# TheoCoombes/ClipCap

Measured on AMD Instinct MI355X. Metric: train samples/sec (512-d prefix, 40-tok caption), higher is better.
Workload: dtype bf16; 1 GPU; BASELINE configs[1]: TransformerMapper(8L,P=L=10,H=8)+frozen GPT-2-small; per_gpu_batch=256, global_batch=256, encoder_dim=512, train_language_model=False, parallelism=dp1

## Files before the change

### clipcap_amd/csrc/gemm.hip.h

```cpp
#pragma once
#include <cstdlib>
#include <type_traits>
#include "common.hip.h"
#include "gemm_api.h"

namespace CC_NS {

constexpr int G_BM = 128, G_BN = 128, G_BK = 64, G_THREADS = 256;
constexpr int G_TILE_BYTES = G_BM * G_BK * 2;
constexpr int G_EPI_LD = 68;

struct GemmShape {
    int M, N, K;
    int lda, ldb;
    int k_chunk;
    int group_m;
    int stagger;
    int flags = 0;
};

__device__ __forceinline__ int g_lds_off(int row, int chunk) {
    return row * 128 + (((chunk ^ (row >> 1) ^ ((row >> 4) & 3)) & 7) << 4);
}

// ... 23 lines not shown
__device__ __forceinline__ void g_load_ks(StageRegs& s, const op16_t* __restrict__ base, int ld, int rows, int r0,
                                          int k0, int kend, int tid) {
    const int ng = (tid & 7) | (((tid >> 4) & 1) << 3);
    const int kg = ((tid >> 3) & 1) | ((tid >> 5) << 1);
    const int r = r0 + ng * 8;
#pragma unroll
    for (int j = 0; j < 4; j++) {
        const int k = k0 + kg * 4 + j;
        if (k < kend && r < rows)
            s.v[j] = *reinterpret_cast<const uint4*>(base + (size_t)k * ld + r);
        else
            s.v[j] = make_uint4(0, 0, 0, 0);
    }
}
__device__ __forceinline__ void l_store_ks(const StageRegs& s, char* lds, int tid) {
    const int ng = (tid & 7) | (((tid >> 4) & 1) << 3);
    const int kg = ((tid >> 3) & 1) | ((tid >> 5) << 1);
    const int kc = kg >> 1, half = (kg & 1) * 8;
    const unsigned in[4][4] = {{s.v[0].x, s.v[0].y, s.v[0].z, s.v[0].w},
                               {s.v[1].x, s.v[1].y, s.v[1].z, s.v[1].w},
                               {s.v[2].x, s.v[2].y, s.v[2].z, s.v[2].w},
                               {s.v[3].x, s.v[3].y, s.v[3].z, s.v[3].w}};
#pragma unroll
    for (int c = 0; c < 4; c++) {
        uint2 ev, od;
        ev.x = __builtin_amdgcn_perm(in[1][c], in[0][c], 0x05040100u);
        ev.y = __builtin_amdgcn_perm(in[3][c], in[2][c], 0x05040100u);
        od.x = __builtin_amdgcn_perm(in[1][c], in[0][c], 0x07060302u);
        od.y = __builtin_amdgcn_perm(in[3][c], in[2][c], 0x07060302u);
        const int n = ng * 8 + 2 * c;
        *reinterpret_cast<uint2*>(lds + g_lds_off(n, kc) + half) = ev;
        *reinterpret_cast<uint2*>(lds + g_lds_off(n + 1, kc) + half) = od;
    }
}

template <int L>
__device__ __forceinline__ void g_load(StageRegs& s, const op16_t* base, int ld, int rows, int r0, int k0, int kend,
                                       int tid) {
    if constexpr (L == 0)
        g_load_kc(s, base, ld, rows, r0, k0, kend, tid);
    else
        g_load_ks(s, base, ld, rows, r0, k0, kend, tid);
}
template <int L>
__device__ __forceinline__ void l_store(const StageRegs& s, char* lds, int tid) {
    if constexpr (L == 0)
        l_store_kc(s, lds, tid);
    else
        l_store_ks(s, lds, tid);
}


template <class E> struct epi_row_strip { static constexpr bool value = false; };
template <class E, class = void> struct epi_acc_init { static constexpr bool value = false; };
template <class E> struct epi_acc_init<E, decltype((void)&E::init4)> { static constexpr bool value = true; };
template <class E, class = void> struct epi_strip_aux { static constexpr bool value = false; typedef char type; };
template <class E> struct epi_strip_aux<E, decltype((void)sizeof(typename E::StripAux))> { static constexpr bool value = true; typedef typename E::StripAux type; };

template <class Epi, int I0 = 0, int I1 = 4>
__device__ __forceinline__ void gemm_epilogue(f32x4 (&acc)[4][4], char* smem, int wave, int lane, int row0, int col0, const Epi& epi) {
    float* strip = reinterpret_cast<float*>(smem) + wave * (16 * G_EPI_LD);
    const int er = (lane >> 4) * 4, ec = lane & 15;
    constexpr bool kAux = epi_strip_aux<Epi>::value;
    typename epi_strip_aux<Epi>::type aux[4][2];
    (void)aux;
    if constexpr (kAux) {
#pragma unroll
        for (int i = I0; i < I1; i++)
#pragma unroll
            for (int s = 0; s < 2; s++) {
                const int q = lane + 64 * s;
                aux[i][s] = epi.load_aux(row0 + i * 16 + (q >> 3), col0 + (q & 7) * 8);
            }
        __builtin_amdgcn_sched_barrier(0);
    }
#pragma unroll
    for (int i = I0; i < I1; i++) {
#pragma unroll
        for (int j = 0; j < 4; j++)
#pragma unroll
            for (int r = 0; r < 4; r++) strip[(er + r) * G_EPI_LD + j * 16 + ec] = acc[i][j][r];
#pragma unroll
        for (int s = 0; s < 2; s++) {
            const int q = lane + 64 * s;
            const int lr = q >> 3, c8 = q & 7;
            float v[8];
            const float4 a = *reinterpret_cast<const float4*>(strip + lr * G_EPI_LD + c8 * 8);
            const float4 b = *reinterpret_cast<const float4*>(strip + lr * G_EPI_LD + c8 * 8 + 4);
            v[0] = a.x; v[1] = a.y; v[2] = a.z; v[3] = a.w; v[4] = b.x; v[5] = b.y; v[6] = b.z; v[7] = b.w;
            if constexpr (kAux) epi(row0 + i * 16 + lr, col0 + c8 * 8, v, aux[i][s]);
            else epi(row0 + i * 16 + lr, col0 + c8 * 8, v);
        }
    }
}

template <class Epi, int NI, int NJ>
__device__ __forceinline__ void gemm_epilogue_regs(f32x4 (&acc)[NI][NJ], int lane, int row0, int col0, const Epi& epi) {
    static_assert(NI % 2 == 0 || NJ % 2 == 0, "leftover column tiles pair along i");
    const int q = lane >> 4, rl = lane & 15;
#define G_PAIR(X, Y, V)                                                                                                  \
    _Pragma("unroll") for (int r_ = 0; r_ < 4; r_++) {                                                                   \
        const auto s_ = __builtin_amdgcn_permlane16_swap(__float_as_uint((X)[r_]), __float_as_uint((Y)[r_]), false, false); \
        (V)[r_] = __uint_as_float(s_[0]);                                                                                \
        (V)[4 + r_] = __uint_as_float(s_[1]);                                                                            \
    }
    if constexpr (epi_row_strip<Epi>::value) {
        static_assert(!epi_row_strip<Epi>::value || NJ == 4, "row-strip epilogues need a 64-column wave strip");
        typename Epi::RowAux tg[NI];
#pragma unroll
        for (int i = 0; i < NI; i++) tg[i] = epi.load_row(row0 + i * 16 + rl);
#pragma unroll
        for (int i = 0; i < NI; i++) {
            float va[8], vb[8];
            G_PAIR(acc[i][0], acc[i][1], va);
            G_PAIR(acc[i][NJ - 2], acc[i][NJ - 1], vb);
            const int cb = col0 + (q & 1) * 16 + (q >> 1) * 8;
            epi.strip(row0 + i * 16 + rl, cb, cb + 32, va, vb, tg[i]);
        }
    } else {
        if constexpr (Epi::kPre) {
#pragma unroll
            for (int i = 0; i < NI; i++)
#pragma unroll
                for (int j = 0; j < NJ; j++) epi.pre4(row0 + i * 16 + rl, col0 + j * 16 + q * 4, acc[i][j]);
        }
        float bias[(NJ + 1) / 2][8];
#pragma unroll
        for (int jp = 0; jp < NJ / 2; jp++) epi.bias8(col0 + (2 * jp + (q & 1)) * 16 + (q >> 1) * 8, bias[jp]);
        if constexpr (NJ & 1) epi.bias8(col0 + (NJ - 1) * 16 + (q >> 1) * 8, bias[NJ / 2]);
        __builtin_amdgcn_sched_barrier(0);
#pragma unroll
        for (int i = 0; i < NI; i++) {
#pragma unroll
            for (int jp = 0; jp < NJ / 2; jp++) {
                float v[8];
                G_PAIR(acc[i][2 * jp], acc[i][2 * jp + 1], v);
                epi.fin(row0 + i * 16 + rl, col0 + (2 * jp + (q & 1)) * 16 + (q >> 1) * 8, v, bias[jp]);
            }
            if constexpr (NJ & 1) {
                if (i & 1) {
                    float v[8];
                    G_PAIR(acc[i - 1][NJ - 1], acc[i][NJ - 1], v);
                    epi.fin(row0 + (i - 1 + (q & 1)) * 16 + rl, col0 + (NJ - 1) * 16 + (q >> 1) * 8, v, bias[NJ / 2]);
                }
            }
        }
    }
#undef G_PAIR
}

__device__ __forceinline__ void tile_coords(int tile, int tiles_m, int tiles_n, int G, int& tm, int& tn) {
    const int band = tile / (G * tiles_n);
    const int first = band * G;
    const int gm = min(G, tiles_m - first);
    const int r = tile - band * G * tiles_n;
    tm = first + r % gm;
    tn = r / gm;
}

__device__ __forceinline__ void acc_zero(f32x4 (&acc)[4][4]) {
#pragma unroll
    for (int i = 0; i < 4; i++)
#pragma unroll
        for (int j = 0; j < 4; j++) acc[i][j] = f32x4{0.f, 0.f, 0.f, 0.f};
}

template <int AL, int BL, class Epi>
__global__ __launch_bounds__(G_THREADS, 2) void gemm_bf16_kernel(const op16_t* __restrict__ A,
                                                                  const op16_t* __restrict__ B, GemmShape g, Epi epi) {
    __shared__ __attribute__((aligned(16))) char smem[4 * G_TILE_BYTES];
    const int tid = threadIdx.x, lane = tid & 63, wave = tid >> 6;
    const int wm = wave >> 1, wn = wave & 1;
    const int tiles_n = (g.N + G_BN - 1) / G_BN, tiles_m = (g.M + G_BM - 1) / G_BM;
// ... 768 lines not shown
                const float* src = part + ((pw * 4 + tile) * 16 + reg) * 64 + ls;
                const float4 x = *reinterpret_cast<const float4*>(src), y = *reinterpret_cast<const float4*>(src + 4);
                v[0] += x.x; v[1] += x.y; v[2] += x.z; v[3] += x.w; v[4] += y.x; v[5] += y.y; v[6] += y.z; v[7] += y.w;
            }
            epi(m0 + row, n0 + c8 * 8, v);
        }
    }
}
static __global__ __launch_bounds__(256) void k_skinny_image(const op16_t* __restrict__ W, op16_t* __restrict__ img, int N, int K) {
    const size_t total = (size_t)N * K / 8;
    const int ktot = K / 64;
    for (size_t e = (size_t)blockIdx.x * 256 + threadIdx.x; e < total; e += (size_t)gridDim.x * 256) {
        const int l = (int)(e & 63);
        size_t f = e >> 6;
        const int i = (int)(f & 1); f >>= 1;
        const int w = (int)(f & 3); f >>= 2;
        const int kt = (int)(f % ktot), tn = (int)(f / ktot);
        const op16_t* src = W + (size_t)(tn * 64 + i * 32 + (l & 31)) * K + kt * 64 + w * 16 + (l >> 5) * 8;
        reinterpret_cast<kb_u32x4*>(img)[e] = *reinterpret_cast<const kb_u32x4*>(src);
    }
}

#endif

#ifndef CC_STAG_READ_FIRST
#define CC_STAG_READ_FIRST 1
#endif
constexpr int H_BM = 256, H_BN = 256, H_BK = 32, H_NS = 4, H_STAGE = (H_BM + H_BN) * H_BK * 2;
__device__ __forceinline__ int h_swz(int row) { return (row & 8) ? 3 : 0; }
__device__ __forceinline__ int h_lds_off(int row, int chunk) { return row * 64 + ((chunk ^ h_swz(row)) << 4); }
__device__ __forceinline__ int h_tt_g(int k) { return (k & 3) | (((k >> 3) & 1) << 2); }
#define H_ISSUE(T, IS_A)                                                                                                 \
    {                                                                                                                    \
        char* st_ = smem + ((T) % H_NS) * SSTAGE + ((IS_A) ? 0 : SBM * H_BK * 2);                                      \
        int k0_ = kbeg + (T)*H_BK;                                                                                       \
        if constexpr (X3F) k0_ = (x3c0_ + ((T) >> 1)) * H_BK + (((T) & 1) ? ((IS_A) ? 2 * x3k_ : x3k_) : 0);    \
        _Pragma("unroll") for (int i_ = 0; i_ < ((IS_A) ? (NI + 1) / 2 : NJ); i_++) {                                        \
            const int seg = (IS_A) ? min(wn + 4 * i_, 2 * NI - 1) : wn + 4 * i_;    \
            const op16_t* src;                                                                                           \
            if constexpr (TT) {                                                                                          \
                const int kr = seg * 2 + (lane >> 5);                                  \
                const int c = (lane & 31) ^ (h_tt_g(kr) << 1);                                                            \
                src = (IS_A) ? A + (size_t)(k0_ + kr) * g.lda + min(m0 + c * 8, g.M - 8)                                  \
                             : B + (size_t)(k0_ + kr) * g.ldb + min(n0 + c * 8, g.N - 8);                                 \
            } else {                                                                                                     \
                const int row = seg * 16 + (lane >> 2);                                   \
                const int chunk = (lane & 3) ^ h_swz(row);                                                               \
                src = (IS_A) ? A + (size_t)min(m0 + row, g.M - 1) * g.lda + k0_ + chunk * 8                               \
                             : B + (size_t)min(n0 + row, g.N - 1) * g.ldb + k0_ + chunk * 8;                              \
            }                                                                                                            \
            __builtin_amdgcn_global_load_lds((gptr_t)src, (lptr_t)(st_ + seg * 1024), 16, 0, 0);                         \
        }                                                                                                                \
    }
typedef __attribute__((ext_vector_type(2))) int h_i32x2;
struct HTTFrag { h_i32x2 lo, hi; };
__device__ __forceinline__ HTTFrag h_tt_read(const char* tile, int lane_base, int xoff) {
    typedef __attribute__((address_space(3))) const char* lp_t;
    const unsigned a = (unsigned)(size_t)(lp_t)(tile + lane_base + xoff);
    HTTFrag f;
    asm volatile("ds_read_b64_tr_b16 %0, %1" : "=v"(f.lo) : "v"(a) : "memory");
    asm volatile("ds_read_b64_tr_b16 %0, %1 offset:2048" : "=v"(f.hi) : "v"(a) : "memory");
    return f;
}
__device__ __forceinline__ op16x8 h_tt_oper(const HTTFrag& f) {
    typedef __attribute__((ext_vector_type(4))) int i32x4_t;
    const i32x4_t v = {f.lo[0], f.lo[1], f.hi[0], f.hi[1]};
    return __builtin_bit_cast(op16x8, v);
}
#define H_LOADF(T)                                                                                                       \
    {                                                                                                                    \
        const char* ca_ = smem + ((T) % H_NS) * SSTAGE;                                                                 \
        const char* cb_ = ca_ + SBM * H_BK * 2;                                                                         \
        if constexpr (TT) {                                                                                              \
            _Pragma("unroll") for (int i_ = 0; i_ < NI; i_++) taf[i_] = h_tt_read(ca_, tt_base, ((grp * 16 + 2 * i_) ^ tt_gx) << 4);  \
            _Pragma("unroll") for (int j_ = 0; j_ < NJ; j_++) tbf[j_] = h_tt_read(cb_, tt_base, ((wn * 8 + 2 * j_) ^ tt_gx) << 4);  \
        } else {                                                                                                         \
            _Pragma("unroll") for (int i_ = 0; i_ < NI; i_++) af[i_] = *reinterpret_cast<const op16x8*>(ca_ + h_lds_off(arow + i_ * 16 + frow, fchunk)); \
            _Pragma("unroll") for (int j_ = 0; j_ < NJ; j_++) bfr[j_] = *reinterpret_cast<const op16x8*>(cb_ + h_lds_off(bcol + j_ * 16 + frow, fchunk)); \
        }                                                                                                                \
    }
#define H_MFMA(T)                                                                                                        \
    {                                                                                                      \
        if constexpr (TT) {                                                                                              \
            _Pragma("unroll") for (int i_ = 0; i_ < NI; i_++) af[i_] = h_tt_oper(taf[i_]);                                 \
            _Pragma("unroll") for (int j_ = 0; j_ < NJ; j_++) bfr[j_] = h_tt_oper(tbf[j_]);                               \
        }                                                                                                                \
        __builtin_amdgcn_s_setprio(1);                                                                                   \
        _Pragma("unroll") for (int i_ = 0; i_ < NI; i_++) _Pragma("unroll") for (int j_ = 0; j_ < NJ; j_++)                \
            acc[i_][j_] = CC_MFMA_16x16x32(bfr[j_], af[i_], acc[i_][j_]);                \
        __builtin_amdgcn_s_setprio(0);                                                                                   \
    }
#define H_LOADF_LO(T)                                                                                                    \
    {                                                                                                                    \
        const char* ca_ = smem + ((T) % H_NS) * SSTAGE;                                                                 \
        const char* cb_ = ca_ + SBM * H_BK * 2;                                                                         \
        _Pragma("unroll") for (int i_ = 0; i_ < NI; i_++) af2[X3F ? i_ : 0] = *reinterpret_cast<const op16x8*>(ca_ + h_lds_off(arow + i_ * 16 + frow, fchunk)); \
        _Pragma("unroll") for (int j_ = 0; j_ < NJ; j_++) bf2[X3F ? j_ : 0] = *reinterpret_cast<const op16x8*>(cb_ + h_lds_off(bcol + j_ * 16 + frow, fchunk)); \
    }
#define H_MFMA_LO()                                                                                                      \
    {                                                                                                                    \
        __builtin_amdgcn_s_setprio(1);                                                                                   \
        _Pragma("unroll") for (int i_ = 0; i_ < NI; i_++) _Pragma("unroll") for (int j_ = 0; j_ < NJ; j_++)                \
            acc[i_][j_] = CC_MFMA_16x16x32(bf2[X3F ? j_ : 0], af[i_], acc[i_][j_]);                                        \
        _Pragma("unroll") for (int i_ = 0; i_ < NI; i_++) _Pragma("unroll") for (int j_ = 0; j_ < NJ; j_++)                \
            acc[i_][j_] = CC_MFMA_16x16x32(bfr[j_], af2[X3F ? i_ : 0], acc[i_][j_]);                                       \
        __builtin_amdgcn_s_setprio(0);                                                                                   \
    }
#define H_SEGEND()                                                                                                       \
    {                                                                                                                    \
        asm volatile("s_waitcnt lgkmcnt(0)" ::: "memory");                                                               \
        __builtin_amdgcn_sched_barrier(0);                                                                               \
        __builtin_amdgcn_s_barrier();                                                                                    \
        __builtin_amdgcn_sched_barrier(0);                                                                               \
    }
#define H_WAIT(T, CNT)                                                                                                   \
    {                                                                                                                    \
        const int rem_ = min(nk - 1, (T) + H_NS - 1) - ((T) + 1);                                                        \
        if (rem_ >= 3) s_wait_vm<3 * (CNT)>();                                                                           \
        else if (rem_ == 2) s_wait_vm<2 * (CNT)>();                                                                      \
        else if (rem_ == 1) s_wait_vm<(CNT)>();                                                                          \
        else s_wait_vm<0>();                                                                                             \
    }
#ifdef CC_STAMP
__device__ unsigned long long cc_stamp_buf[2 * 8];
#define H_STAMP_DECL unsigned long long st_last_ = __builtin_readcyclecounter(), st_acc_[8] = {0, 0, 0, 0, 0, 0, 0, 0};
#define H_STAMP(I) { const unsigned long long n_ = __builtin_readcyclecounter(); st_acc_[I] += n_ - st_last_; st_last_ = n_; }
#define H_STAMP_OUT if (blockIdx.x == 7 && wn == 0 && lane == 0) { for (int i_ = 0; i_ < 8; i_++) cc_stamp_buf[grp * 8 + i_] = st_acc_[i_]; }
#else
#define H_STAMP_DECL
#define H_STAMP(I)
#define H_STAMP_OUT
#endif
template <class Epi, int NJ, bool TT, int NI = 8, bool X3F = false>
__device__ __forceinline__ void gemm_stag256_body(const op16_t* __restrict__ A, const op16_t* __restrict__ B, const GemmShape& g, const Epi& epi,
                                                  int tile, int zslice, char* smem) {
    static_assert(NJ >= 2 && NJ <= 4 && (NI == 8 || NI == 10 || (NI == 5 && NJ == 4)), "wave tile is (16 NI) x (16 NJ)");
    static_assert(!TT || (NJ == 4 && NI == 8), "the K-strided image is laid out for 256 x 256 tiles");
    static_assert(!X3F || (!TT && NJ == 3 && NI == 8), "the fused split-bf16 form is the 256 x 192 NT kernel's");
    constexpr int BN = 64 * NJ, SBM = 32 * NI, SSTAGE = (SBM + H_BN) * H_BK * 2;
    const int tid = threadIdx.x, lane = tid & 63;
    const int wave = __builtin_amdgcn_readfirstlane(tid >> 6);
    const int grp = wave >> 2, wn = wave & 3;
    const int arow = grp * (16 * NI), bcol = wn * (16 * NJ);
    const int tiles_n = (g.N + BN - 1) / BN, tiles_m = (g.M + SBM - 1) / SBM;
    int tm, tn;
    tile_coords(tile, tiles_m, tiles_n, g.group_m, tm, tn);
    const int m0 = tm * SBM, n0 = tn * BN;
    const int kbeg = zslice * g.k_chunk;
    const int x3k_ = g.K / 3;
    const int x3nc_ = x3k_ / H_BK, x3per_ = (x3nc_ + (int)gridDim.z - 1) / (int)gridDim.z;
    const int x3c0_ = zslice * x3per_, x3c1_ = min(x3nc_, x3c0_ + x3per_);
    (void)x3c0_;
    const int nk = X3F ? 2 * max(0, x3c1_ - x3c0_) : (min(g.K, kbeg + g.k_chunk) - kbeg) / H_BK;
    f32x4 acc[NI][NJ];
#pragma unroll
    for (int i = 0; i < NI; i++)
#pragma unroll
        for (int j = 0; j < NJ; j++) acc[i][j] = f32x4{0.f, 0.f, 0.f, 0.f};
    constexpr bool kAccInit = epi_acc_init<Epi>::value && ((NJ == 3 && NI == 8) || NI == 5) && !X3F;
    if constexpr (kAccInit) {
        if (zslice == 0 && epi.init_from_input()) {
            const int q_ = lane >> 4, rl_ = lane & 15;
#pragma unroll
            for (int i = 0; i < NI; i++)
#pragma unroll
                for (int j = 0; j < NJ; j++) epi.init4(m0 + arow + i * 16 + rl_, n0 + bcol + j * 16 + q_ * 4, acc[i][j]);
        }
    }
    op16x8 af[NI], bfr[NJ];
    op16x8 af2[X3F ? NI : 1], bf2[X3F ? NJ : 1];
    (void)af2; (void)bf2;
    HTTFrag taf[TT ? NI : 1], tbf[TT ? NJ : 1];
    (void)taf; (void)tbf;
    const int frow = lane & 15, fchunk = lane >> 4;
    const int tt_base = (8 * fchunk + (frow >> 2)) * 512 + ((frow & 3) >> 1) * 16 + (frow & 1) * 8;
    const int tt_gx = h_tt_g(8 * fchunk + (frow >> 2)) << 1;
    (void)tt_base; (void)tt_gx;
    H_STAMP_DECL
    if constexpr (X3F) {
#define H_G0_STEP(T, LOADF, MFMA)                                                                                        \
        {                                                                                                                \
            LOADF(T);                                                                                                    \
            __builtin_amdgcn_sched_barrier(0);                                                                           \
            if ((T) + H_NS - 1 < nk) H_ISSUE((T) + H_NS - 1, true);                                                      \
            H_SEGEND();                                                                                                  \
            MFMA;                                                                                                        \
            H_WAIT(T, (NI + 1) / 2);                                                                                           \
            H_SEGEND();                                                                                                  \
        }
#define H_G1_STEP(T, LOADF, MFMA_PREV)                                                                                   \
        {                                                                                                                \
            MFMA_PREV;                                                                                                   \
            H_SEGEND();                                                                                                  \
            LOADF(T);                                                                                                    \
            __builtin_amdgcn_sched_barrier(0);                                                                           \
            if ((T) + H_NS - 1 < nk) H_ISSUE((T) + H_NS - 1, false);                                                     \
            H_WAIT(T, NJ);                                                                                               \
            H_SEGEND();                                                                                                  \
        }
        if (grp == 0) {
            if (nk > 0) H_ISSUE(0, true);
            if (nk > 1) H_ISSUE(1, true);
            if (nk > 2) H_ISSUE(2, true);
            H_WAIT(-1, (NI + 1) / 2);
            H_SEGEND();
            for (int t = 0; t < nk; t += 2) {
                H_G0_STEP(t, H_LOADF, H_MFMA(t))
                H_G0_STEP(t + 1, H_LOADF_LO, H_MFMA_LO())
            }
            H_SEGEND();
        } else {
            if (nk > 0) H_ISSUE(0, false);
            if (nk > 1) H_ISSUE(1, false);
            if (nk > 2) H_ISSUE(2, false);
            H_WAIT(-1, NJ);
            H_SEGEND();
            for (int t = 0; t < nk; t += 2) {
                H_G1_STEP(t, H_LOADF, if (t >= 1) H_MFMA_LO())
                H_G1_STEP(t + 1, H_LOADF_LO, H_MFMA(t))
            }
            if (nk > 0) H_MFMA_LO();
            H_SEGEND();
        }
#undef H_G0_STEP
#undef H_G1_STEP
    } else
    if (grp == 0) {
        H_ISSUE(0, true);
        if (nk > 1) H_ISSUE(1, true);
        if (nk > 2) H_ISSUE(2, true);
        if (H_NS > 4 && nk > 3) H_ISSUE(3, true);
        H_WAIT(-1, (NI + 1) / 2);
        H_SEGEND();
        H_STAMP(0)
        for (int t = 0; t < nk; t++) {
#if CC_STAG_READ_FIRST
            H_LOADF(t);
            __builtin_amdgcn_sched_barrier(0);
            if (t + H_NS - 1 < nk) H_ISSUE(t + H_NS - 1, true);
            H_STAMP(1)
#else
            if (t + H_NS - 1 < nk) H_ISSUE(t + H_NS - 1, true);
            H_STAMP(1)
            H_LOADF(t);
#endif
#ifdef CC_STAMP
            asm volatile("s_waitcnt lgkmcnt(0)" ::: "memory");
#endif
            H_STAMP(2)
            H_SEGEND();
            H_STAMP(3)
            H_MFMA(t);
            H_STAMP(4)
            H_WAIT(t, (NI + 1) / 2);
            H_STAMP(5)
            H_SEGEND();
            H_STAMP(6)
        }
        H_SEGEND();
    } else {
        H_ISSUE(0, false);
        if (nk > 1) H_ISSUE(1, false);
        if (nk > 2) H_ISSUE(2, false);
        if (H_NS > 4 && nk > 3) H_ISSUE(3, false);
        H_WAIT(-1, NJ);
        H_SEGEND();
        H_STAMP(0)
        for (int t = 0; t < nk; t++) {
            if (t >= 1) H_MFMA(t - 1);
            H_STAMP(4)
            H_SEGEND();
            H_STAMP(6)
#if CC_STAG_READ_FIRST
            H_LOADF(t);
            __builtin_amdgcn_sched_barrier(0);
            if (t + H_NS - 1 < nk) H_ISSUE(t + H_NS - 1, false);
            H_STAMP(1)
#else
            if (t + H_NS - 1 < nk) H_ISSUE(t + H_NS - 1, false);
            H_STAMP(1)
            H_LOADF(t);
#endif
#ifdef CC_STAMP
            asm volatile("s_waitcnt lgkmcnt(0)" ::: "memory");
#endif
            H_STAMP(2)
            H_WAIT(t, NJ);
            H_STAMP(5)
            H_SEGEND();
            H_STAMP(3)
        }
        H_MFMA(nk - 1); H_SEGEND();
    }
    H_STAMP(0)
    if constexpr (epi_acc_init<Epi>::value && !kAccInit) {
        Epi e2 = epi;
        e2.acc_init = false;
        gemm_epilogue_regs<Epi, NI, NJ>(acc, lane, m0 + arow, n0 + bcol, e2);
    } else {
        gemm_epilogue_regs<Epi, NI, NJ>(acc, lane, m0 + arow, n0 + bcol, epi);
    }
    H_STAMP(7)
    H_STAMP_OUT
}
template <class Epi, int NJ, bool TT = false, int NI = 8, bool X3F = false>
__global__ __launch_bounds__(512, 1) void gemm_nt_stag256_kernel(const op16_t* __restrict__ A, const op16_t* __restrict__ B, GemmShape g, Epi epi) {
    extern __shared__ __attribute__((aligned(1024))) char smem[];
    gemm_stag256_body<Epi, NJ, TT, NI, X3F>(A, B, g, epi, xcd_remap(blockIdx.x, gridDim.x), (int)blockIdx.z, smem);
}
#undef H_STAMP_DECL
#undef H_STAMP
#undef H_STAMP_OUT
#undef H_ISSUE
#undef H_LOADF
#undef H_MFMA
#undef H_LOADF_LO
#undef H_MFMA_LO
#undef H_SEGEND
#undef H_WAIT

#include "gemm_q4.hip.h"

__device__ __forceinline__ HTTFrag g_tt_read(const char* tile, int lane_base, int xoff) {
    typedef __attribute__((address_space(3))) const char* lp_t;
    const unsigned a = (unsigned)(size_t)(lp_t)(tile + lane_base + xoff);
    HTTFrag f;
    asm volatile("ds_read_b64_tr_b16 %0, %1" : "=v"(f.lo) : "v"(a) : "memory");
    asm volatile("ds_read_b64_tr_b16 %0, %1 offset:1024" : "=v"(f.hi) : "v"(a) : "memory");
    return f;
}
__device__ __forceinline__ void glds_tile_tt(const op16_t* __restrict__ base, int ld, int cols, int c0, int k0, char* lds, int wave, int lane) {
#pragma unroll
    for (int i = 0; i < 4; i++) {
        const int seg = wave + 4 * i;
        const int kr = seg * 4 + (lane >> 4);
        const int c = (lane & 15) ^ (h_tt_g(kr) << 1);
        const op16_t* src = base + (size_t)(k0 + kr) * ld + min(c0 + c * 8, cols - 8);
        __builtin_amdgcn_global_load_lds((gptr_t)src, (lptr_t)(lds + seg * 1024), 16, 0, 0);
    }
}
template <class Epi>
__device__ __forceinline__ void gemm_tt_glds4_body(const op16_t* __restrict__ A, const op16_t* __restrict__ B, const GemmShape& g, const Epi& epi,
                                                   int tile, int zslice, char* smemt) {
    const int tid = threadIdx.x, lane = tid & 63;
    const int wave = __builtin_amdgcn_readfirstlane(tid >> 6);
    const int wm = wave >> 1, wn = wave & 1;
    const int tiles_n = (g.N + G_BN - 1) / G_BN, tiles_m = (g.M + G_BM - 1) / G_BM;
    int tm, tn;
    tile_coords(tile, tiles_m, tiles_n, g.group_m, tm, tn);
    const int m0 = tm * G_BM, n0 = tn * G_BN;
    const int kbeg = zslice * g.k_chunk;
    const int nk = (min(g.K, kbeg + g.k_chunk) - kbeg) / G_BK;
    f32x4 acc[4][4];
#pragma unroll
    for (int i = 0; i < 4; i++)
#pragma unroll
        for (int j = 0; j < 4; j++) acc[i][j] = f32x4{0.f, 0.f, 0.f, 0.f};
#define GT_ISSUE(T)                                                                                                      \
    {                                                                                                                    \
        char* st_ = smemt + ((T) & 3) * 2 * G_TILE_BYTES;                                                                \
        glds_tile_tt(A, g.lda, g.M, m0, kbeg + (T)*G_BK, st_, wave, lane);                                               \
        glds_tile_tt(B, g.ldb, g.N, n0, kbeg + (T)*G_BK, st_ + G_TILE_BYTES, wave, lane);                                \
    }
    GT_ISSUE(0);
    if (nk > 1) GT_ISSUE(1);
    if (nk > 2) GT_ISSUE(2);
// ... 266 lines not shown
        *reinterpret_cast<float4*>(p) = make_float4(v[0] + b[0], v[1] + b[1], v[2] + b[2], v[3] + b[3]);
        *reinterpret_cast<float4*>(p + 4) = make_float4(v[4] + b[4], v[5] + b[5], v[6] + b[6], v[7] + b[7]);
    }
};

template <int ACT = -1>
struct EpiDActT {
    act_t* C;
    const act_t* aux;
    int ldc, M, Ns;
    int act;
    int img = 0;
    __device__ __forceinline__ int act_() const { return ACT >= 0 ? ACT : act; }
    __device__ __forceinline__ void operator()(int row, int col, float (&v)[8]) const {
        if (row >= M || col >= Ns) return;
        const size_t o = (size_t)row * ldc + col;
        float a[8];
        act_ld8(aux + o, a);
        if (act_() == 1) {
#pragma unroll
            for (int e = 0; e < 8; e++) v[e] = a[e] > 0.f ? v[e] : 0.f;
        } else if (act_() == 3) {
#pragma unroll
            for (int e = 0; e < 8; e++) v[e] *= a[e];
        } else {
#pragma unroll
            for (int e = 0; e < 8; e++) v[e] *= gelu_new_grad(a[e]);
        }
        epi_store8(C, ldc, row, col, v, img);
    }
    typedef act_raw8 StripAux;
    __device__ __forceinline__ act_raw8 load_aux(int row, int col) const {
        return (row < M && col < Ns) ? act_ldraw8(aux + (size_t)row * ldc + col) : act_zero8();
    }
    __device__ __forceinline__ void operator()(int row, int col, float (&v)[8], const act_raw8& ax) const {
        if (row >= M || col >= Ns) return;
        float a[8];
        act_unpack8(ax, a);
        if (act_() == 1) {
#pragma unroll
            for (int e = 0; e < 8; e++) v[e] = a[e] > 0.f ? v[e] : 0.f;
        } else if (act_() == 3) {
#pragma unroll
            for (int e = 0; e < 8; e++) v[e] *= a[e];
        } else {
#pragma unroll
            for (int e = 0; e < 8; e++) v[e] *= gelu_new_grad(a[e]);
        }
        epi_store8(C, ldc, row, col, v, img);
    }
    static constexpr bool kPre = true;
    __device__ __forceinline__ void pre4(int row, int col, f32x4& a) const {
        if (row >= M || col >= Ns) return;
        float x[4];
        act_unpack4(act_ldraw4(aux + (size_t)row * ldc + col), x[0], x[1], x[2], x[3]);
#pragma unroll
        for (int e = 0; e < 4; e++) a[e] = act_() == 1 ? (x[e] > 0.f ? a[e] : 0.f) : (act_() == 3 ? a[e] * x[e] : a[e] * gelu_new_grad(x[e]));
    }
    __device__ __forceinline__ void bias8(int, float (&b)[8]) const {
#pragma unroll
        for (int e = 0; e < 8; e++) b[e] = 0.f;
    }
    __device__ __forceinline__ void fin(int row, int col, float (&v)[8], const float (&)[8]) const {
        if (row >= M || col >= Ns) return;
        epi_store8(C, ldc, row, col, v, img);
    }
};
using EpiDAct = EpiDActT<>;
template <class E> struct epi_is_dact { static constexpr bool value = false; };
template <int A> struct epi_is_dact<EpiDActT<A>> { static constexpr bool value = true; };

template <int LO, int HI>
__device__ __forceinline__ float xor_max(float m) {
#pragma unroll
    for (int d = LO; d <= HI; d <<= 1) m = fmaxf(m, __shfl_xor(m, d, 64));
    return m;
}
template <int LO, int HI>
__device__ __forceinline__ float xor_sum(float s) {
#pragma unroll
    for (int d = LO; d <= HI; d <<= 1) s += __shfl_xor(s, d, 64);
    return s;
}
__device__ __forceinline__ void row_stats8(int col, int V, const float (&v)[8], float& m, float& s) {
    m = -INFINITY;
#pragma unroll
    for (int e = 0; e < 8; e++)
        if (col + e < V) m = fmaxf(m, v[e]);
    m = xor_max<1, 4>(m);
    s = 0.f;
#pragma unroll
    for (int e = 0; e < 8; e++)
        if (col + e < V) s += __expf(v[e] - m);
    s = xor_sum<1, 4>(s);
}
template <bool ZERO_PAD, bool FAST>
__device__ __forceinline__ void row_stats_strip(int ca, int cb, int V, float (&va)[8], float (&vb)[8], float& m, float& s) {
    constexpr float L2E = 1.4426950408889634f;
    s = 0.f;
    if (FAST && __builtin_amdgcn_readfirstlane(ca | 63) < V) {
        m = fmaxf(fmaxf(fmaxf(va[0], va[1]), fmaxf(va[2], va[3])), fmaxf(fmaxf(va[4], va[5]), fmaxf(va[6], va[7])));
        m = fmaxf(m, fmaxf(fmaxf(fmaxf(vb[0], vb[1]), fmaxf(vb[2], vb[3])), fmaxf(fmaxf(vb[4], vb[5]), fmaxf(vb[6], vb[7]))));
        m = xor_max<16, 32>(m);
        const float ml = -m * L2E;
#pragma unroll
        for (int e = 0; e < 8; e++) s += __builtin_amdgcn_exp2f(fmaf(va[e], L2E, ml)) + __builtin_amdgcn_exp2f(fmaf(vb[e], L2E, ml));
    } else {
        m = -INFINITY;
#pragma unroll
        for (int e = 0; e < 8; e++) {
            if (ca + e >= V) { if (ZERO_PAD) va[e] = 0.f; } else m = fmaxf(m, va[e]);
            if (cb + e >= V) { if (ZERO_PAD) vb[e] = 0.f; } else m = fmaxf(m, vb[e]);
        }
        m = xor_max<16, 32>(m);
#pragma unroll
        for (int e = 0; e < 8; e++) {
            if (ca + e < V) s += __expf(va[e] - m);
            if (cb + e < V) s += __expf(vb[e] - m);
        }
    }
    s = xor_sum<16, 32>(s);
}
template <class E>
// ... 171 lines not shown
};
template <> struct epi_row_strip<EpiLogits> { static constexpr bool value = true; };
template <> struct epi_row_strip<EpiLMHead> { static constexpr bool value = true; };
template <> struct epi_row_strip<EpiLMHeadScore> { static constexpr bool value = true; };
template <> struct epi_row_strip<EpiLMHeadExp> { static constexpr bool value = true; };

template <auto Kernel, class... Args>
inline void launch_dyn(dim3 grid, dim3 block, size_t shmem, hipStream_t st, const Args&... args) {
    static bool attr = false;
    if (!attr) { (void)hipFuncSetAttribute((const void*)Kernel, hipFuncAttributeMaxDynamicSharedMemorySize, (int)shmem); attr = true; }
    hipLaunchKernelGGL(Kernel, grid, block, shmem, st, args...);
}
template <class Epi>
inline int launch_gemm_s64(const op16_t* A, int lda, const op16_t* B, int ldb, int M, int N, int K, int ksplit, int nj, const Epi& epi, int* ks_eff,
                           hipStream_t st, const op16_t* Bimg = nullptr);
inline bool x3_fused_on() {
    static const bool on = kX3 && !(cc_lab_env("CC_X3_FUSED") && atoi(cc_lab_env("CC_X3_FUSED")) == 0);
    return on;
}
template <class Epi>
inline int launch_gemm(int al, int bl, const op16_t* A, int lda, const op16_t* B, int ldb, int M, int N, int K,
                       int ksplit, const Epi& epi, hipStream_t st, int tile = -2, int group_m = 0) {
    if (M <= 0 || N <= 0 || K <= 0) return CC_OK;
    if ((lda & 7) || (ldb & 7) || ((uintptr_t)A & 15) || ((uintptr_t)B & 15)) return CC_ERR_SHAPE;
    if (al == 0 && (K & 7)) return CC_ERR_SHAPE;
    if (bl == 0 && (K & 7)) return CC_ERR_SHAPE;
    if (al == 1 && (M & 7)) return CC_ERR_SHAPE;
    if (bl == 1 && (N & 7)) return CC_ERR_SHAPE;
    if constexpr (!epi_row_strip<Epi>::value && !epi_strip_aux<Epi>::value) {
        if (g_gemm_s64 > 0 && al == 0 && bl == 0 && (K % G_BK) == 0 && M <= 1024)
            return launch_gemm_s64(A, lda, B, ldb, M, N, K, ksplit, g_gemm_s64, epi, nullptr, st);
    }
    GemmShape g;
    g.M = M; g.N = N; g.K = K; g.lda = lda; g.ldb = ldb;
    static const int env_group = []() { const char* e = cc_lab_env("CC_GROUP_M"); return e ? atoi(e) : 0; }();
    g.group_m = env_group > 0 ? env_group : (group_m > 0 ? group_m : 8);
    static const int env_stagger = []() { const char* e = cc_lab_env("CC_GEMM_STAGGER"); return e ? atoi(e) : 0; }();
    g.stagger = env_stagger;
    if (ksplit < 1) ksplit = 1;
    int kt = (K + G_BK - 1) / G_BK;
    int per = (kt + ksplit - 1) / ksplit;
    ksplit = (kt + per - 1) / per;
    g.k_chunk = per * G_BK;
    dim3 grid(((M + G_BM - 1) / G_BM) * ((N + G_BN - 1) / G_BN), 1, ksplit);
    const int s256 = tile != -2 ? tile : g_gemm_tile_mode;
    int nj = 0, ni = 8;
    constexpr bool can160 = !kX3 && !epi_row_strip<Epi>::value && !epi_is_dact<Epi>::value;
    constexpr bool zsplit_ok = std::is_same<Epi, EpiF32>::value;
    if (al == 0 && bl == 0 && (K % H_BK) == 0 && (ksplit == 1 || (zsplit_ok && tile > 0)) && s256 != 0) {
        const long tm = (M + H_BM - 1) / H_BM, t128 = (long)grid.x;
        const long t256 = tm * ((N + 255) / 256), t192 = tm * ((N + 191) / 192), t320 = (long)((M + 319) / 320) * ((N + 255) / 256);
        const double c128 = t128 <= 256 ? 16384.0 / 0.75 : (double)((t128 + 511) / 512) * 32768.0;
        const double c256 = (double)((t256 + 255) / 256) * 65536.0 / 1.2, c192 = (double)((t192 + 255) / 256) * 49152.0 / 1.15;
        const double c320 = (double)((t320 + 255) / 256) * 81920.0 / 1.3;
        constexpr bool can192 = !epi_row_strip<Epi>::value;
        constexpr bool can320 = !epi_is_dact<Epi>::value;
        const long t160 = (long)((M + 159) / 160) * ((N + 255) / 256);
        const double c160 = (double)((t160 + 255) / 256) * 40960.0 / 1.1;
        static const bool s160_on = []() { const char* e = cc_lab_env("CC_GEMM_S160"); return !e || atoi(e) != 0; }();
        if (can160 && (s256 == 6 || s256 == 7 || (s256 < 0 && s160_on && ksplit == 1 && c160 < 0.98 * c128 && c160 < 0.98 * c256 && c160 < 0.98 * c320 && (!can192 || c160 < 0.98 * c192)))) { nj = 4; ni = 5; }
        else if (s256 == 5 || (can320 && s256 < 0 && c320 < 0.98 * c128 && c320 < c256 && (!can192 || c320 < c192))) { nj = 4; ni = 10; }
        else if (s256 == 4 || (s256 < 0 && c256 < 0.98 * c128 && (!can192 || c256 <= c192))) nj = 4;
        else if (can192 && (s256 == 3 || (s256 < 0 && c192 < 0.98 * c128))) nj = 3;
    }
    if (nj) {
        const int bm = 32 * ni;
        const size_t sh = (size_t)H_NS * (bm + H_BN) * H_BK * 2;
        const dim3 gr((unsigned)(((M + bm - 1) / bm) * ((N + 64 * nj - 1) / (64 * nj))), 1, (unsigned)ksplit);
        if (nj == 4 && ni == 8) launch_dyn<gemm_nt_stag256_kernel<Epi, 4, false, 8>>(gr, dim3(512), sh, st, A, B, g, epi);
        else if (nj == 4 && ni == 5) {
            if constexpr (can160) {
                static const bool q4_on = []() { const char* e = cc_lab_env("CC_GEMM_Q4"); return !e || atoi(e) != 0; }();
                const bool fits32 = (size_t)M * (size_t)lda * 2 < 0xffff0000ull && (size_t)N * (size_t)ldb * 2 < 0xffff0000ull;
                const int ns = (K % 192 == 0 && K >= 384) ? 3 : ((K % 128 == 0 && K >= 256) ? 2 : 0);
                static const bool q4_last = []() { const char* e = cc_lab_env("CC_Q4_LAST"); return !e || atoi(e) != 0; }();
                g.flags = q4_last ? 0 : 1;
                if (ns && fits32 && ksplit == 1 && s256 != 6 && (q4_on || s256 == 7)) {
                    static const int ncu = []() { int n = 0, dev = 0; (void)hipGetDevice(&dev); (void)hipDeviceGetAttribute(&n, hipDeviceAttributeMultiprocessorCount, dev); return n > 0 ? n : 256; }();
                    const int tiles = ((M + 159) / 160) * ((N + 255) / 256);
                    const dim3 gq((unsigned)(tiles < ncu ? tiles : ncu));
                    if (ns == 3) {
                        launch_dyn<gemm_nt_q4_kernel<Epi, 5, 3>>(gq, dim3(256), (size_t)3 * (160 + 256) * 128, st, A, B, g, epi);
                    } else {
                        launch_dyn<gemm_nt_q4_kernel<Epi, 5, 2>>(gq, dim3(256), (size_t)2 * (160 + 256) * 128, st, A, B, g, epi);
                    }
                } else launch_dyn<gemm_nt_stag256_kernel<Epi, 4, false, 5>>(gr, dim3(512), sh, st, A, B, g, epi);
            }
        }
        else if (nj == 4) launch_dyn<gemm_nt_stag256_kernel<Epi, 4, false, 10>>(gr, dim3(512), sh, st, A, B, g, epi);
        else if constexpr (!epi_row_strip<Epi>::value) {
            bool fused = false;
            if constexpr (kX3) {
                const bool x3f_on = x3_fused_on();
                if (x3f_on && (K % (3 * H_BK)) == 0 && ksplit <= K / (3 * H_BK)) {
                    launch_dyn<gemm_nt_stag256_kernel<Epi, 3, false, 8, true>>(gr, dim3(512), sh, st, A, B, g, epi);
                    fused = true;
                }
            }
            if (!fused) launch_dyn<gemm_nt_stag256_kernel<Epi, 3, false, 8>>(gr, dim3(512), sh, st, A, B, g, epi);
        }
    } else
#ifdef CC_GEMM_ABLATION
    static const int abl = []() { const char* e = cc_lab_env("CC_GEMM_ABL"); return e ? atoi(e) : 0; }();
    if (al == 0 && bl == 0 && (K % G_BK) == 0 && abl == 1) { hipLaunchKernelGGL((gemm_nt_glds_kernel<Epi, 1>), grid, dim3(G_THREADS), 0, st, A, B, g, epi); }
    else if (al == 0 && bl == 0 && (K % G_BK) == 0 && abl == 2) { hipLaunchKernelGGL((gemm_nt_glds_kernel<Epi, 2>), grid, dim3(G_THREADS), 0, st, A, B, g, epi); }
    else if (al == 0 && bl == 0 && (K % G_BK) == 0 && abl == 4) { hipLaunchKernelGGL((gemm_nt_glds_kernel<Epi, 4>), grid, dim3(G_THREADS), 0, st, A, B, g, epi); }
    else if (al == 0 && bl == 0 && (K % G_BK) == 0 && abl == 5) { hipLaunchKernelGGL((gemm_nt_glds_kernel<Epi, 5>), grid, dim3(G_THREADS), 0, st, A, B, g, epi); }
    else if (al == 0 && bl == 0 && (K % G_BK) == 0 && abl == 6) { hipLaunchKernelGGL((gemm_nt_glds_kernel<Epi, 6>), grid, dim3(G_THREADS), 0, st, A, B, g, epi); }
    else
#endif
    if (al == 0 && bl == 0 && (K % G_BK) == 0 && (long)grid.x * grid.z <= 256 && g_gemm_tile_mode != 0 && K / (int)grid.z >= 4 * G_BK) {
        constexpr size_t sh4 = (size_t)8 * G_TILE_BYTES;
        bool fused = false;
        if constexpr (kX3) {
            const bool x3f_on = x3_fused_on();
            if (g_gemm_small_x2 && x3f_on && ksplit == 1 && (K % (3 * G_BK)) == 0) {
                launch_dyn<gemm_nt_glds4x2_x3f_kernel<Epi>>(grid, dim3(2 * G_THREADS), sh4, st, A, B, g, epi);
                fused = true;
            }
        }
        if (fused) {}
        else if (g_gemm_small_x2) launch_dyn<gemm_nt_glds4x2_kernel<Epi>>(grid, dim3(2 * G_THREADS), sh4, st, A, B, g, epi);
// ... 207 lines not shown
```

### clipcap_amd/csrc/gemm_inst_dact.hip

```cpp
#include "gemm.hip.h"
#include "gemm_api.h"
namespace CC_NS {
int gemm_dact(int al, int bl, ActIn A, int lda, const op16_t* B, int ldb, int M, int N, int K, Act Co, int ldc,
              const act_t* aux, int act, Call& cx) {
    const hipStream_t st = cx.st;
    act_t* const C = Co.p;
    cc_shared::ProfScope _all(cc_shared::SITE_ALL_GEMMS, st, 2.0 * M * N * (double)K);
    if ((ldc & 7) || (N & 7)) return CC_ERR_SHAPE;
    const op16_t* A16;
    const int rca = nt_operand(cx, A, al, bl, M, lda, ldb, K, A16);
    if (rca != CC_OK) return rca;
    EpiDAct e{C, aux, ldc, M, N, act};
    e.img = Co.img;
    static const bool spec_on = []() { const char* v = cc_lab_env("CC_EPI_SPEC"); return !v || atoi(v) != 0; }();
    if (spec_on && act == 3 && e.img == 0) {
        EpiDActT<3> m{C, aux, ldc, M, N, 3};
        return launch_gemm(al, bl, A16, lda, B, ldb, M, N, K, 1, m, st);
    }
    return launch_gemm(al, bl, A16, lda, B, ldb, M, N, K, 1, e, st);
}
}
```

Measured before the change: 22140 samples/s.

## Prefetch dact aux tile into LDS through phantom pipeline stages in stag256 GEMM

For the activation-gradient GEMM epilogue, the aux (pre-activation) tile is now streamed into the freed LDS pipeline stages with global_load_lds during the final K iterations, so the epilogue multiply reads from LDS instead of issuing scattered global loads after the main loop. It also re-enables the 320-row tile for dact epilogues when staging is on and changes that tile's cost weight. The added waits and extra issue logic may stall the tail of the mainloop, and the staging path only applies to NT, 256-wide, single-split launches with 16-byte-aligned aux.

```diff
diff --git a/clipcap_amd/csrc/gemm.hip.h b/clipcap_amd/csrc/gemm.hip.h
--- a/clipcap_amd/csrc/gemm.hip.h
+++ b/clipcap_amd/csrc/gemm.hip.h
@@ -99,6 +99,7 @@
 
 
 template <class E> struct epi_row_strip { static constexpr bool value = false; };
+template <class E> struct epi_lds_aux { static constexpr bool value = false; };
 template <class E, class = void> struct epi_acc_init { static constexpr bool value = false; };
 template <class E> struct epi_acc_init<E, decltype((void)&E::init4)> { static constexpr bool value = true; };
 template <class E, class = void> struct epi_strip_aux { static constexpr bool value = false; typedef char type; };
@@ -141,7 +142,7 @@
     }
 }
 
-template <class Epi, int NI, int NJ>
+template <class Epi, int NI, int NJ, bool PRE_DONE = false>
 __device__ __forceinline__ void gemm_epilogue_regs(f32x4 (&acc)[NI][NJ], int lane, int row0, int col0, const Epi& epi) {
     static_assert(NI % 2 == 0 || NJ % 2 == 0, "leftover column tiles pair along i");
     const int q = lane >> 4, rl = lane & 15;
@@ -165,7 +166,7 @@
             epi.strip(row0 + i * 16 + rl, cb, cb + 32, va, vb, tg[i]);
         }
     } else {
-        if constexpr (Epi::kPre) {
+        if constexpr (Epi::kPre && !PRE_DONE) {
 #pragma unroll
             for (int i = 0; i < NI; i++)
 #pragma unroll
@@ -1040,6 +1041,24 @@
             __builtin_amdgcn_global_load_lds((gptr_t)src, (lptr_t)(st_ + seg * 1024), 16, 0, 0);                         \
         }                                                                                                                \
     }
+#define H_ISSUE_AUX(P, IS_A)                                                                                             \
+    {                                                                                                                    \
+        char* st_ = smem + ((nk + (P)) % H_NS) * SSTAGE + ((IS_A) ? 0 : SBM * H_BK * 2);                                \
+        _Pragma("unroll") for (int i_ = 0; i_ < ((IS_A) ? NI / 2 : NJ); i_++) {                                          \
+            const int seg = wn + 4 * i_;                                                                                 \
+            const int blk_ = (P) * (SSTAGE / 512) + ((IS_A) ? 0 : 4 * NI) + 2 * seg + (lane >> 5);                        \
+            const int w_ = blk_ & 7, n_ = blk_ >> 3;                                                                      \
+            const int row = m0 + (w_ >> 2) * (16 * NI) + (n_ / NJ) * 16 + (lane & 15);                                    \
+            const int col = n0 + (w_ & 3) * (16 * NJ) + (n_ % NJ) * 16 + ((lane >> 4) & 1) * 8;                           \
+            const act_t* src = epi.aux + (size_t)min(row, epi.M - 1) * epi.ldc + min(col, epi.Ns - 8);                   \
+            __builtin_amdgcn_global_load_lds((gptr_t)src, (lptr_t)(st_ + seg * 1024), 16, 0, 0);                         \
+        }                                                                                                                \
+    }
+#define H_ISSUE_T(T, IS_A)                                                                                               \
+    {                                                                                                                    \
+        if ((T) < nk) H_ISSUE(T, IS_A)                                                                                   \
+        else if constexpr (AUXS) H_ISSUE_AUX((T) - nk, IS_A)                                                             \
+    }
 typedef __attribute__((ext_vector_type(2))) int h_i32x2;
 struct HTTFrag { h_i32x2 lo, hi; };
 __device__ __forceinline__ HTTFrag h_tt_read(const char* tile, int lane_base, int xoff) {
@@ -1103,23 +1122,44 @@
     }
 #define H_WAIT(T, CNT)                                                                                                   \
     {                                                                                                                    \
-        const int rem_ = min(nk - 1, (T) + H_NS - 1) - ((T) + 1);                                                        \
-        if (rem_ >= 3) s_wait_vm<3 * (CNT)>();                                                                           \
+        const int rem_ = min(nkw - 1, (T) + H_NS - 1) - ((T) + 1);    \
+        if (AUXS) s_wait_vm<(H_NS - 2) * (CNT)>();                                                                       \
+        else if (rem_ >= 3) s_wait_vm<3 * (CNT)>();                                                                      \
         else if (rem_ == 2) s_wait_vm<2 * (CNT)>();                                                                      \
         else if (rem_ == 1) s_wait_vm<(CNT)>();                                                                          \
         else s_wait_vm<0>();                                                                                             \
     }
+template <class Epi, int NI, int NJ, int NST>
+__device__ __forceinline__ void h_aux_apply(f32x4 (&acc)[NI][NJ], const Epi& epi, int lane, int wave, int row0, int col0, const char* b0,
+                                            const char* b1, const char* b2) {
+    static_assert(H_NS == 4 && NST % 3 == 0 && NST <= NI * NJ, "three phantom tiles, NST / 3 blocks per wave in each");
+    constexpr int PW = NST / 3, NDIR = NI * NJ - NST;
+    const int q = lane >> 4, rl = lane & 15;
+    act_raw4 far[NDIR];
+#pragma unroll
+    for (int n = NST; n < NI * NJ; n++) far[n - NST] = epi.ld4(row0 + (n / NJ) * 16 + rl, col0 + (n % NJ) * 16 + q * 4);
+    const int slot = (wave * 64 + (q >> 1) * 32 + 2 * rl + (q & 1)) * 8;
+#pragma unroll
+    for (int n = 0; n < NST; n++) {
+        const char* b = n / PW == 0 ? b0 : (n / PW == 1 ? b1 : b2);
+        epi.mul4(*reinterpret_cast<const act_raw4*>(b + (n % PW) * 4096 + slot), acc[n / NJ][n % NJ]);
+    }
+#pragma unroll
+    for (int n = NST; n < NI * NJ; n++) epi.mul4(far[n - NST], acc[n / NJ][n % NJ]);
+}
 #ifdef CC_STAMP
 __device__ unsigned long long cc_stamp_buf[2 * 8];
 #define H_STAMP_DECL unsigned long long st_last_ = __builtin_readcyclecounter(), st_acc_[8] = {0, 0, 0, 0, 0, 0, 0, 0};
 #define H_STAMP(I) { const unsigned long long n_ = __builtin_readcyclecounter(); st_acc_[I] += n_ - st_last_; st_last_ = n_; }
+#define H_STAMP_LGKM asm volatile("s_waitcnt lgkmcnt(0)" ::: "memory");
 #define H_STAMP_OUT if (blockIdx.x == 7 && wn == 0 && lane == 0) { for (int i_ = 0; i_ < 8; i_++) cc_stamp_buf[grp * 8 + i_] = st_acc_[i_]; }
 #else
 #define H_STAMP_DECL
 #define H_STAMP(I)
+#define H_STAMP_LGKM
 #define H_STAMP_OUT
 #endif
-template <class Epi, int NJ, bool TT, int NI = 8, bool X3F = false>
+template <class Epi, int NJ, bool TT, int NI = 8, bool X3F = false, bool AUXS = false>
 __device__ __forceinline__ void gemm_stag256_body(const op16_t* __restrict__ A, const op16_t* __restrict__ B, const GemmShape& g, const Epi& epi,
                                                   int tile, int zslice, char* smem) {
     static_assert(NJ >= 2 && NJ <= 4 && (NI == 8 || NI == 10 || (NI == 5 && NJ == 4)), "wave tile is (16 NI) x (16 NJ)");
@@ -1155,6 +1195,8 @@
                 for (int j = 0; j < NJ; j++) epi.init4(m0 + arow + i * 16 + rl_, n0 + bcol + j * 16 + q_ * 4, acc[i][j]);
         }
     }
+    static_assert(!AUXS || (epi_lds_aux<Epi>::value && !TT && !X3F && NJ == 4 && (NI == 8 || NI == 10)), "phantom tiles: NT, 256 wide, 16-bit aux");
+    const int nkw = nk + (AUXS ? H_NS - 1 : 0);
     op16x8 af[NI], bfr[NJ];
     op16x8 af2[X3F ? NI : 1], bf2[X3F ? NJ : 1];
     (void)af2; (void)bf2;
@@ -1215,91 +1257,142 @@
     } else
     if (grp == 0) {
         H_ISSUE(0, true);
-        if (nk > 1) H_ISSUE(1, true);
-        if (nk > 2) H_ISSUE(2, true);
+        H_ISSUE_T(1, true);
+        H_ISSUE_T(2, true);
         if (H_NS > 4 && nk > 3) H_ISSUE(3, true);
         H_WAIT(-1, (NI + 1) / 2);
         H_SEGEND();
         H_STAMP(0)
-        for (int t = 0; t < nk; t++) {
 #if CC_STAG_READ_FIRST
-            H_LOADF(t);
-            __builtin_amdgcn_sched_barrier(0);
-            if (t + H_NS - 1 < nk) H_ISSUE(t + H_NS - 1, true);
-            H_STAMP(1)
+#define H_S0_STEP(T, ISSUE)                                                                                              \
+        {                                                                                                                \
+            H_LOADF(T);                                                                                                  \
+            __builtin_amdgcn_sched_barrier(0);                                                                           \
+            ISSUE;                                                                                                       \
+            H_STAMP(1)                                                                                                   \
+            H_STAMP_LGKM                                                                                                 \
+            H_STAMP(2)                                                                        \
+            H_SEGEND();                                                                                                  \
+            H_STAMP(3)                                                                \
+            H_MFMA(T);                                                                                                   \
+            H_STAMP(4)                                                                                   \
+            H_WAIT(T, (NI + 1) / 2);                                                                                     \
+            H_STAMP(5)                                                                                   \
+            H_SEGEND();                                                                                                  \
+            H_STAMP(6)                                                                \
+        }
 #else
-            if (t + H_NS - 1 < nk) H_ISSUE(t + H_NS - 1, true);
-            H_STAMP(1)
-            H_LOADF(t);
+#define H_S0_STEP(T, ISSUE)                                                                                              \
+        {                                                                                                                \
+            ISSUE;                                      \
+            H_STAMP(1)                                                                                    \
+            H_LOADF(T);                                                                                                  \
+            H_STAMP_LGKM                                                                                                 \
+            H_STAMP(2)                                                                                                   \
+            H_SEGEND();                                                                                                  \
+            H_STAMP(3)                                                                                                   \
+            H_MFMA(T);                                                                                                   \
+            H_STAMP(4)                                                                                                   \
+            H_WAIT(T, (NI + 1) / 2);                                                                                     \
+            H_STAMP(5)                                                                                                   \
+            H_SEGEND();                                                                                                  \
+            H_STAMP(6)                                                                                                   \
+        }
 #endif
-#ifdef CC_STAMP
-            asm volatile("s_waitcnt lgkmcnt(0)" ::: "memory");
-#endif
-            H_STAMP(2)
-            H_SEGEND();
-            H_STAMP(3)
-            H_MFMA(t);
-            H_STAMP(4)
-            H_WAIT(t, (NI + 1) / 2);
-            H_STAMP(5)
-            H_SEGEND();
-            H_STAMP(6)
+        if constexpr (AUXS) {
+            const int nmain = max(nk - (H_NS - 1), 0);
+            for (int t = 0; t < nmain; t++) H_S0_STEP(t, H_ISSUE(t + H_NS - 1, true))
+            for (int t = nmain; t < nk; t++) H_S0_STEP(t, H_ISSUE_AUX(t + H_NS - 1 - nk, true))
+            s_wait_vm<0>();
+        } else {
+            for (int t = 0; t < nk; t++) H_S0_STEP(t, if (t + H_NS - 1 < nk) H_ISSUE(t + H_NS - 1, true))
         }
         H_SEGEND();
     } else {
         H_ISSUE(0, false);
-        if (nk > 1) H_ISSUE(1, false);
-        if (nk > 2) H_ISSUE(2, false);
+        H_ISSUE_T(1, false);
+        H_ISSUE_T(2, false);
         if (H_NS > 4 && nk > 3) H_ISSUE(3, false);
         H_WAIT(-1, NJ);
         H_SEGEND();
         H_STAMP(0)
-        for (int t = 0; t < nk; t++) {
-            if (t >= 1) H_MFMA(t - 1);
-            H_STAMP(4)
-            H_SEGEND();
-            H_STAMP(6)
 #if CC_STAG_READ_FIRST
-            H_LOADF(t);
-            __builtin_amdgcn_sched_barrier(0);
-            if (t + H_NS - 1 < nk) H_ISSUE(t + H_NS - 1, false);
-            H_STAMP(1)
+#define H_S1_STEP(T, ISSUE)                                                                                              \
+        {                                                                                                                \
+            if ((T) >= 1) H_MFMA((T) - 1);                                                                               \
+            H_STAMP(4)                                                                                                   \
+            H_SEGEND();                                                                                                  \
+            H_STAMP(6)                                                                                                   \
+            H_LOADF(T);                                                                                                  \
+            __builtin_amdgcn_sched_barrier(0);                                                                           \
+            ISSUE;                                                                                                       \
+            H_STAMP(1)                                                                                                   \
+            H_STAMP_LGKM                                                                                                 \
+            H_STAMP(2)                                                                                                   \
+            H_WAIT(T, NJ);                                                                                               \
+            H_STAMP(5)                                                                                                   \
+            H_SEGEND();                                                                                                  \
+            H_STAMP(3)                                                                                                   \
+        }
 #else
-            if (t + H_NS - 1 < nk) H_ISSUE(t + H_NS - 1, false);
-            H_STAMP(1)
-            H_LOADF(t);
+#define H_S1_STEP(T, ISSUE)                                                                                              \
+        {                                                                                                                \
+            if ((T) >= 1) H_MFMA((T) - 1);                                                                               \
+            H_STAMP(4)                                                                                                   \
+            H_SEGEND();                                                                                                  \
+            H_STAMP(6)                                                                                                   \
+            ISSUE;                                                \
+            H_STAMP(1)                                                                                                   \
+            H_LOADF(T);                                                                                                  \
+            H_STAMP_LGKM                                                                                                 \
+            H_STAMP(2)                                                                                                   \
+            H_WAIT(T, NJ);                                                                                               \
+            H_STAMP(5)                                                                                                   \
+            H_SEGEND();                                                                                                  \
+            H_STAMP(3)                                                                                                   \
+        }
 #endif
-#ifdef CC_STAMP
-            asm volatile("s_waitcnt lgkmcnt(0)" ::: "memory");
-#endif
-            H_STAMP(2)
-            H_WAIT(t, NJ);
-            H_STAMP(5)
-            H_SEGEND();
-            H_STAMP(3)
-        }
-        H_MFMA(nk - 1); H_SEGEND();
-    }
+        if constexpr (AUXS) {
+            const int nmain = max(nk - (H_NS - 1), 0);
+            for (int t = 0; t < nmain; t++) H_S1_STEP(t, H_ISSUE(t + H_NS - 1, false))
+            for (int t = nmain; t < nk; t++) H_S1_STEP(t, H_ISSUE_AUX(t + H_NS - 1 - nk, false))
+            H_MFMA(nk - 1);
+            s_wait_vm<0>();
+        } else {
+            for (int t = 0; t < nk; t++) H_S1_STEP(t, if (t + H_NS - 1 < nk) H_ISSUE(t + H_NS - 1, false))
+            H_MFMA(nk - 1);
+        }
+        H_SEGEND();
+    }
+#undef H_S0_STEP
+#undef H_S1_STEP
     H_STAMP(0)
     if constexpr (epi_acc_init<Epi>::value && !kAccInit) {
         Epi e2 = epi;
         e2.acc_init = false;
         gemm_epilogue_regs<Epi, NI, NJ>(acc, lane, m0 + arow, n0 + bcol, e2);
+    } else if constexpr (AUXS) {
+        h_aux_apply<Epi, NI, NJ, 3 * SSTAGE / 4096>(acc, epi, lane, wave, m0 + arow, n0 + bcol, smem + (nk % H_NS) * SSTAGE,
+                                                    smem + ((nk + 1) % H_NS) * SSTAGE, smem + ((nk + 2) % H_NS) * SSTAGE);
+        gemm_epilogue_regs<Epi, NI, NJ, true>(acc, lane, m0 + arow, n0 + bcol, epi);
     } else {
         gemm_epilogue_regs<Epi, NI, NJ>(acc, lane, m0 + arow, n0 + bcol, epi);
     }
     H_STAMP(7)
     H_STAMP_OUT
 }
-template <class Epi, int NJ, bool TT = false, int NI = 8, bool X3F = false>
+template <class Epi, int NJ, bool TT = false, int NI = 8, bool X3F = false, bool AUXS = false>
 __global__ __launch_bounds__(512, 1) void gemm_nt_stag256_kernel(const op16_t* __restrict__ A, const op16_t* __restrict__ B, GemmShape g, Epi epi) {
     extern __shared__ __attribute__((aligned(1024))) char smem[];
-    gemm_stag256_body<Epi, NJ, TT, NI, X3F>(A, B, g, epi, xcd_remap(blockIdx.x, gridDim.x), (int)blockIdx.z, smem);
+    gemm_stag256_body<Epi, NJ, TT, NI, X3F, AUXS>(A, B, g, epi, xcd_remap(blockIdx.x, gridDim.x), (int)blockIdx.z, smem);
 }
 #undef H_STAMP_DECL
 #undef H_STAMP
+#undef H_STAMP_LGKM
 #undef H_STAMP_OUT
 #undef H_ISSUE
+#undef H_ISSUE_AUX
+#undef H_ISSUE_T
 #undef H_LOADF
 #undef H_MFMA
 #undef H_LOADF_LO
@@ -1672,8 +1765,13 @@
     static constexpr bool kPre = true;
     __device__ __forceinline__ void pre4(int row, int col, f32x4& a) const {
         if (row >= M || col >= Ns) return;
+        mul4(act_ldraw4(aux + (size_t)row * ldc + col), a);
+    }
+    bool lds_stage = false;
+    __device__ __forceinline__ act_raw4 ld4(int row, int col) const { return act_ldraw4(aux + (size_t)min(row, M - 1) * ldc + min(col, Ns - 4)); }
+    __device__ __forceinline__ void mul4(const act_raw4& r, f32x4& a) const {
         float x[4];
-        act_unpack4(act_ldraw4(aux + (size_t)row * ldc + col), x[0], x[1], x[2], x[3]);
+        act_unpack4(r, x[0], x[1], x[2], x[3]);
 #pragma unroll
         for (int e = 0; e < 4; e++) a[e] = act_() == 1 ? (x[e] > 0.f ? a[e] : 0.f) : (act_() == 3 ? a[e] * x[e] : a[e] * gelu_new_grad(x[e]));
     }
@@ -1689,6 +1787,7 @@
 using EpiDAct = EpiDActT<>;
 template <class E> struct epi_is_dact { static constexpr bool value = false; };
 template <int A> struct epi_is_dact<EpiDActT<A>> { static constexpr bool value = true; };
+template <int A> struct epi_lds_aux<EpiDActT<A>> { static constexpr bool value = !kX3; };
 
 template <int LO, int HI>
 __device__ __forceinline__ float xor_max(float m) {
@@ -1966,9 +2065,10 @@
         const long t256 = tm * ((N + 255) / 256), t192 = tm * ((N + 191) / 192), t320 = (long)((M + 319) / 320) * ((N + 255) / 256);
         const double c128 = t128 <= 256 ? 16384.0 / 0.75 : (double)((t128 + 511) / 512) * 32768.0;
         const double c256 = (double)((t256 + 255) / 256) * 65536.0 / 1.2, c192 = (double)((t192 + 255) / 256) * 49152.0 / 1.15;
-        const double c320 = (double)((t320 + 255) / 256) * 81920.0 / 1.3;
+        const double c320 = (double)((t320 + 255) / 256) * 81920.0 / (epi_is_dact<Epi>::value ? 1.1 : 1.3);
         constexpr bool can192 = !epi_row_strip<Epi>::value;
-        constexpr bool can320 = !epi_is_dact<Epi>::value;
+        bool can320 = !epi_is_dact<Epi>::value;
+        if constexpr (epi_lds_aux<Epi>::value) can320 = epi.lds_stage;
         const long t160 = (long)((M + 159) / 160) * ((N + 255) / 256);
         const double c160 = (double)((t160 + 255) / 256) * 40960.0 / 1.1;
         static const bool s160_on = []() { const char* e = cc_lab_env("CC_GEMM_S160"); return !e || atoi(e) != 0; }();
@@ -1981,7 +2081,16 @@
         const int bm = 32 * ni;
         const size_t sh = (size_t)H_NS * (bm + H_BN) * H_BK * 2;
         const dim3 gr((unsigned)(((M + bm - 1) / bm) * ((N + 64 * nj - 1) / (64 * nj))), 1, (unsigned)ksplit);
-        if (nj == 4 && ni == 8) launch_dyn<gemm_nt_stag256_kernel<Epi, 4, false, 8>>(gr, dim3(512), sh, st, A, B, g, epi);
+        bool staged = false;
+        if constexpr (epi_lds_aux<Epi>::value) {
+            if (epi.lds_stage && nj == 4 && (ni == 8 || ni == 10) && ksplit == 1) {
+                if (ni == 8) launch_dyn<gemm_nt_stag256_kernel<Epi, 4, false, 8, false, true>>(gr, dim3(512), sh, st, A, B, g, epi);
+                else launch_dyn<gemm_nt_stag256_kernel<Epi, 4, false, 10, false, true>>(gr, dim3(512), sh, st, A, B, g, epi);
+                staged = true;
+            }
+        }
+        if (staged) {}
+        else if (nj == 4 && ni == 8) launch_dyn<gemm_nt_stag256_kernel<Epi, 4, false, 8>>(gr, dim3(512), sh, st, A, B, g, epi);
         else if (nj == 4 && ni == 5) {
             if constexpr (can160) {
                 static const bool q4_on = []() { const char* e = cc_lab_env("CC_GEMM_Q4"); return !e || atoi(e) != 0; }();
diff --git a/clipcap_amd/csrc/gemm_inst_dact.hip b/clipcap_amd/csrc/gemm_inst_dact.hip
--- a/clipcap_amd/csrc/gemm_inst_dact.hip
+++ b/clipcap_amd/csrc/gemm_inst_dact.hip
@@ -12,9 +12,12 @@
     if (rca != CC_OK) return rca;
     EpiDAct e{C, aux, ldc, M, N, act};
     e.img = Co.img;
+    static const bool stage_on = []() { const char* v = cc_lab_env("CC_DACT_STAGE"); return !v || atoi(v) != 0; }();
+    e.lds_stage = stage_on && !kX3 && ((uintptr_t)aux & 15) == 0;
     static const bool spec_on = []() { const char* v = cc_lab_env("CC_EPI_SPEC"); return !v || atoi(v) != 0; }();
     if (spec_on && act == 3 && e.img == 0) {
         EpiDActT<3> m{C, aux, ldc, M, N, 3};
+        m.lds_stage = e.lds_stage;
         return launch_gemm(al, bl, A16, lda, B, ldb, M, N, K, 1, m, st);
     }
     return launch_gemm(al, bl, A16, lda, B, ldb, M, N, K, 1, e, st);
```

Measured after the change: 22300 samples/s (median of 6 runs). No clear change (+0.7%).
